# mathwrx/Decouple-and-Couple_Learning_in_Multi-Modal_Brain_Tumor_Segmentation

Measured on AMD Instinct MI355X. Metric: training volumes/sec (4x128^3), higher is better.
Workload: dtype bf16x3 forward (split-bf16 MFMA operands hi.hi+hi.lo+lo.hi: logits within 1e-3 of the fp32 reference) / bf16 data-gradient / bf16 weight-gradient MFMA operands; f32 accumulate, f32 storage, f32 master weights

## Files before the change

### decouple-and-couple_learning_in_multi-modal_brain_tumor_segmentation_amd/csrc/conv_args.h

```cpp
#pragma once
#include "common.h"

typedef __bf16 bf16x8 __attribute__((ext_vector_type(8)));
typedef unsigned u32x4 __attribute__((ext_vector_type(4)));

struct ConvArgsB {
  ConvGeom g;
  const float* x; const uint4* wpk; const float* bias; float* y;
  const float* in_scale; const float* in_shift; float in_slope;
  const float* residual; int r_ldc; const float* out_scale; double* stats;
  unsigned long long unused_[2];
  const float* nb_x; int nb_ldc; const float* nb_scale; const float* nb_shift; float nb_slope;
  int groups, x_goff, y_goff;
  const uint4* wpk_g[3]; const float* bias_g[3];
  const uint4* x16; const uint4* zero16;
  unsigned short* y16;
};

typedef __bf16 bf16x2_t __attribute__((ext_vector_type(2)));
typedef float f32x2_t __attribute__((ext_vector_type(2)));
__device__ __forceinline__ unsigned pack_bf16(float a, float b) {
  const f32x2_t f = {a, b};
  return __builtin_bit_cast(unsigned, __builtin_convertvector(f, bf16x2_t));
}
__device__ __forceinline__ float bf16_round(float a) { return (float)(__bf16)a; }
__device__ __forceinline__ void split_bf16(float a, float b, unsigned& hi, unsigned& lo) {
  hi = pack_bf16(a, b);
  const float ha = __builtin_bit_cast(float, hi << 16), hb = __builtin_bit_cast(float, hi & 0xffff0000u);
  lo = pack_bf16(a - ha, b - hb);
}
__device__ __forceinline__ float act01(float v, float slope) { return fmaxf(v, v * slope); }


static inline int cfg_extent(int op, int Di, int Hi, int Wi, int Do, int Ho, int Wo, int cd[3]) {
  cd[0] = Do; cd[1] = Ho; cd[2] = Wo;
  if (op == CWF_CONVT2) { cd[0] = Di; cd[1] = Hi; cd[2] = Wi; return 8; }
  if (op == CWF_CONV3_S2_DGRAD) { cd[0] = (Do + 1) / 2; cd[1] = (Ho + 1) / 2; cd[2] = (Wo + 1) / 2; return 8; }
  return 1;
}

int cwf_try_conv_ws(int op, int x3, ConvArgsB& a, hipStream_t st, int* rc);

int conv_fp32_launch(const cwf_conv_args& d, hipStream_t st);
int conv_stem_launch(const cwf_conv_args& d, hipStream_t st);
int conv_s2c16_launch(const cwf_conv_args& d, hipStream_t st);
int wgrad_fp32_launch(const cwf_wgrad_args& d, int* nsplit_used, hipStream_t st);
```

### decouple-and-couple_learning_in_multi-modal_brain_tumor_segmentation_amd/csrc/conv_bf16.hip

```cpp
#include "common.h"
#include <cstdio>
#include <cstdlib>
#include <type_traits>

#include "conv_args.h"

#define CB_MAXS 13
struct StageSlots { int goff[CB_MAXS]; unsigned inb; int nslots; };

__device__ __forceinline__ void stage_slots_init(StageSlots& ss, const ConvGeom& g, int id0, int ih0, int iw0, int tid) {
  const int nvox_in = g.ID * g.IH * g.IW;
  ss.nslots = (nvox_in + 63) >> 6; ss.inb = 0u;
  const int dq = 64 / g.IW, dr = 64 - dq * g.IW;
  int iw = (tid >> 2) % g.IW, t2 = (tid >> 2) / g.IW;
  int ih = t2 % g.IH, idd = t2 / g.IH;
#pragma unroll
  for (int i = 0; i < CB_MAXS; ++i) {
    const int v = (tid >> 2) + 64 * i;
    const int gd = id0 + idd, gh = ih0 + ih, gw = iw0 + iw;
    const bool ok = v < nvox_in && gd >= 0 && gd < g.Di && gh >= 0 && gh < g.Hi && gw >= 0 && gw < g.Wi;
    ss.goff[i] = ok ? ((gd * g.Hi + gh) * g.Wi + gw) * g.x_ldc : 0;
    ss.inb |= ok ? (1u << i) : 0u;
    iw += dr; int adv = dq;
    if (iw >= g.IW) { iw -= g.IW; ++adv; }
// ... 997 lines not shown
}

__global__ void gather_split_bf16_kernel(const cwf_gather_desc* __restrict__ table) {
  const cwf_gather_desc d = table[blockIdx.y];
  unsigned short* dst = reinterpret_cast<unsigned short*>(d.dst);
  const int64_t ngrp = d.n >> 3;
  const bool vec = ((d.n & 7) == 0) && ((reinterpret_cast<uintptr_t>(d.map) & 15) == 0) && ((reinterpret_cast<uintptr_t>(d.dst) & 15) == 0);
  if (vec) {
    for (int64_t gi = (int64_t)blockIdx.x * blockDim.x + threadIdx.x; gi < ngrp; gi += (int64_t)gridDim.x * blockDim.x) {
      const int4 m0 = *reinterpret_cast<const int4*>(d.map + gi * 8), m1 = *reinterpret_cast<const int4*>(d.map + gi * 8 + 4);
      const int mm[8] = {m0.x, m0.y, m0.z, m0.w, m1.x, m1.y, m1.z, m1.w};
      bool other = false;
#pragma unroll
      for (int e = 0; e < 8; ++e) other |= mm[e] == -2;
      unsigned short hh[8], ll[8];
#pragma unroll
      for (int e = 0; e < 8; ++e) {
        const float v = mm[e] >= 0 ? d.src[mm[e]] : 0.f;
        const __bf16 h = (__bf16)v;
        const __bf16 l = (__bf16)(v - (float)h);
        hh[e] = __builtin_bit_cast(unsigned short, h); ll[e] = __builtin_bit_cast(unsigned short, l);
      }
      unsigned short* o = dst + gi * 16;
      if (!other) {
        uint4 H, L;
        H.x = hh[0] | ((unsigned)hh[1] << 16); H.y = hh[2] | ((unsigned)hh[3] << 16); H.z = hh[4] | ((unsigned)hh[5] << 16); H.w = hh[6] | ((unsigned)hh[7] << 16);
        L.x = ll[0] | ((unsigned)ll[1] << 16); L.y = ll[2] | ((unsigned)ll[3] << 16); L.z = ll[4] | ((unsigned)ll[5] << 16); L.w = ll[6] | ((unsigned)ll[7] << 16);
        *reinterpret_cast<uint4*>(o) = H;
        *reinterpret_cast<uint4*>(o + 8) = L;
      } else {
#pragma unroll
        for (int e = 0; e < 8; ++e)
          if (mm[e] != -2) { o[e] = hh[e]; o[e + 8] = ll[e]; }
      }
    }
    return;
  }
  for (int64_t i = (int64_t)blockIdx.x * blockDim.x + threadIdx.x; i < d.n; i += (int64_t)gridDim.x * blockDim.x) {
    const int32_t m = d.map[i];
    if (m == -2) continue;
    const float v = m >= 0 ? d.src[m] : 0.f;
    const __bf16 h = (__bf16)v;
    const __bf16 l = (__bf16)(v - (float)h);
    const int64_t o = (i >> 3) * 16 + (i & 7);
    dst[o] = __builtin_bit_cast(unsigned short, h);
    dst[o + 8] = __builtin_bit_cast(unsigned short, l);
  }
}

extern "C" int cwf_gather_split_bf16(const struct cwf_gather_desc* table, int nlayers, int64_t max_n, void* stream) {
  if (!table || nlayers <= 0 || max_n <= 0) return CWF_E_BADARG;
  int64_t gx = cdiv64(max_n, 8 * 256); if (gx > 256) gx = 256; if (gx < 1) gx = 1;
  hipLaunchKernelGGL(gather_split_bf16_kernel, dim3((unsigned)gx, nlayers), dim3(256), 0, cwf_stream(stream), table);
  CWF_LAUNCH_CHECK();
  return 0;
}

namespace {
struct TileCfg { int MT, NT, WM; };
TileCfg choose_cfg(int op, const int cdims[3], int ncls, int N, int ntiles) {
  const bool s2 = (op == CWF_CONV3_S2 || op == CWF_CONVT2_DGRAD);
  static const TileCfg all[] = {{4, 4, 1}, {2, 4, 2}, {2, 4, 4}, {4, 2, 4}, {4, 1, 4}, {1, 4, 4}, {1, 2, 4}, {1, 2, 2}, {1, 1, 4}};
  TileCfg best = {1, 1, 4};
  double best_score = -1.0;
  for (const TileCfg& c : all) {
    const int WN = 4 / c.WM, MTOT = c.MT * c.WM, NTOT = c.NT * WN;
    if (s2 && MTOT > 4) continue;
    int TD, TH;
    switch (MTOT) { case 16: TD = 4; TH = 4; break; case 8: TD = 2; TH = 4; break; case 4: TD = 2; TH = 2; break; case 2: TD = 1; TH = 2; break; default: TD = 1; TH = 1; }
    const double sp_tiles = (double)cdiv(cdims[0], TD) * cdiv(cdims[1], TH) * cdiv(cdims[2], 16);
    const double sp_eff = ((double)cdims[0] * cdims[1] * cdims[2]) / (sp_tiles * MTOT * 16);
    const int ngrp = cdiv(ntiles, NTOT);
    const double n_eff = (double)ntiles / (ngrp * NTOT);
    const double nwg = sp_tiles * ngrp * N * ncls;
    const double fill = nwg >= 512 ? 1.0 : nwg / 512.0;
    const double reuse = 1.0 - 0.35 / (c.MT * c.NT) - 0.1 / MTOT;
    const double score = sp_eff * n_eff * fill * reuse;
    if (score > best_score) { best_score = score; best = c; }
  }
  return best;
}

template <int MT, int NT, int WM, bool X3>
int launch_cfg(const ConvArgsB& a, hipStream_t st) {
  constexpr int WN = 4 / WM;
  const ConvGeom& g = a.g;
  const size_t lds_tile = (size_t)g.ID * g.IH * g.IW * 16 * sizeof(unsigned short) * (X3 ? 2 : 1);
  const size_t lds_red = (size_t)4 * NT * 16 * 2 * sizeof(float);
  const size_t lds = lds_tile > lds_red ? lds_tile : lds_red;
  if (lds > 160 * 1024) return CWF_E_TOOLARGE;
  CWF_MAX_LDS_ONCE((&conv_bf16_kernel<MT, NT, WM, X3>));
  dim3 grid(g.tiles_d * g.tiles_h * g.tiles_w, cdiv(g.ntiles, WN * NT), g.N * g.ncls * (a.groups ? a.groups : 1));
  hipLaunchKernelGGL((conv_bf16_kernel<MT, NT, WM, X3>), grid, dim3(256), lds, st, a);
  CWF_LAUNCH_CHECK();
  return 0;
}
}

extern "C" int cwf_debug_conv_bf16_cfg(int op, int N, int Di, int Hi, int Wi, int Do, int Ho, int Wo, int Cout, int* mt_nt_wm) {
  if (!mt_nt_wm || N <= 0 || Di <= 0 || Hi <= 0 || Wi <= 0 || Do <= 0 || Ho <= 0 || Wo <= 0 || Cout <= 0 || op < CWF_CONV3_S1 ||
      op > CWF_CONVT2_DGRAD)
    return CWF_E_BADARG;
  int cd[3];
  const int ncls = cfg_extent(op, Di, Hi, Wi, Do, Ho, Wo, cd);
  const TileCfg c = choose_cfg(op, cd, ncls, N, cdiv(Cout, 16));
  mt_nt_wm[0] = c.MT; mt_nt_wm[1] = c.NT; mt_nt_wm[2] = c.WM;
  return 0;
}

static void c16_tap_order(ConvGeom& g) {
  int nat[27];
  for (int t = 0; t < 27; ++t) nat[t] = g.tapofs[t];
  for (int t = 0; t < 27; ++t) g.tapofs[t] = nat[c16_tap(t)];
}

static int conv_bf16_impl(const cwf_conv_args& d, hipStream_t st) {
  const int op = d.op, x3 = d.precision == CWF_BF16X3, N = d.N, Cin = d.Cin, Cout = d.Cout, y_ldc = d.y_ldc;
  const float* x = d.x16 ? reinterpret_cast<const float*>(d.x16) : d.x;
  const int x_ldc = d.x16 ? 16 : d.x_ldc;
  if (!x || !d.wpk || !d.y || N <= 0 || Cin <= 0 || Cout <= 0) return CWF_E_BADARG;
  if (d.nb_x && (!d.stats || !d.nb_scale || !d.nb_shift || d.nb_ldc < Cout)) return CWF_E_BADARG;
  if ((Cin & 3) || (x_ldc & 3) || x_ldc < Cin || y_ldc < Cout) return CWF_E_ALIGN;
  if (((uintptr_t)x & 15) || ((uintptr_t)d.wpk & 15)) return CWF_E_ALIGN;
  if (d.in_scale && !d.in_shift) return CWF_E_BADARG;
  ConvArgsB a;
  int cd[3];
  const int ncls = cfg_extent(op, d.Di, d.Hi, d.Wi, d.Do, d.Ho, d.Wo, cd);
  const TileCfg c = choose_cfg(op, cd, ncls, N, cdiv(Cout, 16));
  int rc = cwf_build_geom(a.g, op, N, d.Di, d.Hi, d.Wi, Cin, x_ldc, d.Do, d.Ho, d.Wo, Cout, y_ldc, c.MT * c.WM);
  if (rc) return rc;
  a.x = x; a.wpk = reinterpret_cast<const uint4*>(d.wpk); a.bias = d.bias; a.y = d.y; a.in_scale = d.in_scale; a.in_shift = d.in_shift;
  a.in_slope = d.x16 ? 1.f : d.in_slope; a.residual = d.residual; a.r_ldc = d.r_ldc; a.out_scale = d.out_scale; a.stats = d.stats;
  a.nb_x = d.nb_x; a.nb_ldc = d.nb_ldc; a.nb_scale = d.nb_scale; a.nb_shift = d.nb_shift; a.nb_slope = d.nb_x ? d.nb_slope : 1.f;
  a.groups = 0; a.x_goff = 0; a.y_goff = 0;
  a.x16 = reinterpret_cast<const uint4*>(d.x16); a.zero16 = reinterpret_cast<const uint4*>(d.zero16);
  a.y16 = reinterpret_cast<unsigned short*>(d.y16);
  for (int q = 0; q < 3; ++q) { a.wpk_g[q] = nullptr; a.bias_g[q] = nullptr; }
  if (d.x16) {
    c16_tap_order(a.g);
    rc = cwf_build_geom(a.g, op, N, d.Di, d.Hi, d.Wi, Cin, x_ldc, d.Do, d.Ho, d.Wo, Cout, y_ldc, 16);
    if (rc) return rc;
    return launch_conv16s<false, true>(a, st);
  }
  {
    int ks, nt;
    if (pw_eligible(op, a, &ks, &nt)) {
      if (d.y16 && (op != CWF_CONV1 || (Cout & 3) || ((uintptr_t)d.y16 & 7))) return CWF_E_BADARG;
      return x3 ? dispatch_pw<true>(op, a, st, ks, nt) : dispatch_pw<false>(op, a, st, ks, nt);
    }
    if (d.y16) return CWF_E_BADARG;
  }
  {
    int rcw = 0;
    if (cwf_try_conv_ws(op, x3, a, st, &rcw)) return rcw;
  }
  if (op == CWF_CONV3_S1 && Cin <= 16 && Cout <= 16) c16_tap_order(a.g);
  if (op == CWF_CONV3_S1 && Cin <= 16 && Cout <= 16 && (int64_t)d.Do * d.Ho * d.Wo >= 32768) {
    rc = cwf_build_geom(a.g, op, N, d.Di, d.Hi, d.Wi, Cin, x_ldc, d.Do, d.Ho, d.Wo, Cout, y_ldc, 16);
    if (rc) return rc;
    return x3 ? launch_conv16s<true>(a, st) : launch_conv16s<false>(a, st);
  }
#define CWF_CFG(mt, nt, wm) if (c.MT == mt && c.NT == nt && c.WM == wm) return x3 ? launch_cfg<mt, nt, wm, true>(a, st) : launch_cfg<mt, nt, wm, false>(a, st);
  CWF_CFG(4, 4, 1) CWF_CFG(2, 4, 2) CWF_CFG(2, 4, 4) CWF_CFG(4, 2, 4) CWF_CFG(4, 1, 4)
  CWF_CFG(1, 4, 4) CWF_CFG(1, 2, 4) CWF_CFG(1, 2, 2) CWF_CFG(1, 1, 4)
#undef CWF_CFG
  return CWF_E_BADARG;
}

static int conv_grouped_impl(const cwf_conv_args& d, hipStream_t st) {
  const int op = d.op, x3 = d.precision == CWF_BF16X3, groups = d.groups, N = d.N, Cin = d.Cin, Cout = d.Cout;
  const int x_ldc = d.x_ldc, y_ldc = d.y_ldc, x_goff = d.x_goff, y_goff = d.y_goff;
  if (!d.x || !d.y || N <= 0 || Cin <= 0 || Cout <= 0) return CWF_E_BADARG;
  if ((Cin & 3) || (x_ldc & 3) || (x_goff & 3) || x_ldc < (groups - 1) * x_goff + Cin || y_ldc < (groups - 1) * y_goff + Cout) return CWF_E_ALIGN;
  if ((uintptr_t)d.x & 15) return CWF_E_ALIGN;
  ConvArgsB a;
  int cd[3];
  TileCfg c = choose_cfg(op, cd, cfg_extent(op, d.Di, d.Hi, d.Wi, d.Do, d.Ho, d.Wo, cd), N * groups, cdiv(Cout, 16));
  int rc = cwf_build_geom(a.g, op, N, d.Di, d.Hi, d.Wi, Cin, x_ldc, d.Do, d.Ho, d.Wo, Cout, y_ldc, c.MT * c.WM);
  if (rc) return rc;
  a.x = d.x; a.wpk = nullptr; a.bias = nullptr; a.y = d.y; a.in_scale = nullptr; a.in_shift = nullptr; a.in_slope = 1.f;
  a.residual = nullptr; a.r_ldc = 0; a.out_scale = nullptr; a.stats = nullptr;
  a.nb_x = nullptr; a.nb_ldc = 0; a.nb_scale = nullptr; a.nb_shift = nullptr; a.nb_slope = 1.f;
  a.groups = groups; a.x_goff = x_goff; a.y_goff = y_goff;
  a.x16 = nullptr; a.zero16 = nullptr; a.y16 = nullptr;
  for (int q = 0; q < 3; ++q) {
    a.wpk_g[q] = q < groups ? reinterpret_cast<const uint4*>(d.wpk_g[q]) : nullptr;
    a.bias_g[q] = q < groups ? d.bias_g[q] : nullptr;
    if (q < groups && (!d.wpk_g[q] || ((uintptr_t)d.wpk_g[q] & 15))) return CWF_E_ALIGN;
  }
  if (Cin <= 16 && Cout <= 16) c16_tap_order(a.g);
#define CWF_CFG(mt, nt, wm) if (c.MT == mt && c.NT == nt && c.WM == wm) return x3 ? launch_cfg<mt, nt, wm, true>(a, st) : launch_cfg<mt, nt, wm, false>(a, st);
  CWF_CFG(4, 4, 1) CWF_CFG(2, 4, 2) CWF_CFG(2, 4, 4) CWF_CFG(4, 2, 4) CWF_CFG(4, 1, 4)
  CWF_CFG(1, 4, 4) CWF_CFG(1, 2, 4) CWF_CFG(1, 2, 2) CWF_CFG(1, 1, 4)
#undef CWF_CFG
  return CWF_E_BADARG;
}

extern "C" int cwf_conv(const struct cwf_conv_args* args, void* stream) {
  if (!args) return CWF_E_BADARG;
  const cwf_conv_args& d = *args;
  if (d.precision != CWF_FP32 && d.precision != CWF_BF16X3 && d.precision != CWF_BF16) return CWF_E_BADARG;
  const bool fp32 = d.precision == CWF_FP32;
  hipStream_t st = cwf_stream(stream);
  if (d.groups) {
    if (d.groups < 2 || d.groups > 3 || d.op != CWF_CONV3_S1 || d.in_scale || d.residual || d.out_scale || d.stats || d.nb_x || d.x16 ||
        d.y16 || d.w_raw)
      return CWF_E_BADARG;
    if (!fp32) return conv_grouped_impl(d, st);
    for (int q = 0; q < d.groups; ++q) {
      cwf_conv_args g = d;
      g.groups = 0; g.x = d.x + q * d.x_goff; g.y = d.y + q * d.y_goff; g.wpk = d.wpk_g[q]; g.bias = d.bias_g[q];
      const int rc = conv_fp32_launch(g, st);
      if (rc) return rc;
    }
    return 0;
  }
  if (d.x16) {
    if (d.precision != CWF_BF16 || d.in_scale || d.out_scale || d.y16 || !d.zero16 || ((uintptr_t)d.x16 & 15) || ((uintptr_t)d.zero16 & 15))
      return CWF_E_BADARG;
    if (d.op != CWF_CONV3_S1 || d.Cin != 16 || d.Cout != 16 || d.Do != d.Di || d.Ho != d.Hi || d.Wo != d.Wi ||
        (int64_t)d.Di * d.Hi * d.Wi < 32768 || (int64_t)d.N * d.Di * d.Hi * d.Wi >= (1ll << 30))
      return CWF_E_BADARG;
    return conv_bf16_impl(d, st);
  }
  if (d.y16) {
    if (d.nb_x || d.out_scale) return CWF_E_BADARG;
    if (!fp32 && d.op == CWF_CONV1) {
      const int rc = conv_bf16_impl(d, st);
      if (rc != CWF_E_BADARG) return rc;
    }
    cwf_conv_args f = d;
    f.y16 = nullptr;
    const int rc = cwf_conv(&f, stream);
    if (rc) return rc;
    return cwf_to_bf16(d.y, d.y_ldc, nullptr, nullptr, 1.f, d.y16, d.N, (int64_t)d.Do * d.Ho * d.Wo, d.Cout, stream);
  }
  const int64_t vo = (int64_t)d.Do * d.Ho * d.Wo;
  if (d.w_raw && !fp32 && !d.in_scale && !d.residual && !d.nb_x) {
    if (d.op == CWF_CONV3_S1 && d.Cin == 4 && d.Cout == 16 && vo >= 32768) return conv_stem_launch(d, st);
    if (d.op == CWF_CONV3_S2 && d.Cin == 16 && d.Cout == 32 && !d.out_scale && vo >= 32768 &&
        d.Do == (d.Di + 1) / 2 && d.Ho == (d.Hi + 1) / 2 && d.Wo == (d.Wi + 1) / 2)
      return conv_s2c16_launch(d, st);
  }
  if (fp32) return d.nb_x ? CWF_E_BADARG : conv_fp32_launch(d, st);
  return conv_bf16_impl(d, st);
}
```

### decouple-and-couple_learning_in_multi-modal_brain_tumor_segmentation_amd/csrc/conv_ws.hip

```cpp
#include "conv_args.h"
#include <cstdlib>
#include <type_traits>

#define WS_ID 6
#define WS_IH 6
#define WS_IW 18
#define WS_NVOX (WS_ID * WS_IH * WS_IW)
#define WS_SLOTS 11
#define WS_NT 2

struct WsWork { int ngroups, slots, tiles, xcd_perm; };

__host__ __device__ constexpr int ws_tap_bytes(int t) { return (((t / 9) * WS_IH + (t / 3) % 3) * WS_IW + t % 3) * 32; }

template <bool X3>
__global__ __launch_bounds__(512) void convws_kernel(const ConvArgsB a, const WsWork wk) {
  constexpr int NT = WS_NT;
  constexpr int T = 1;
  extern __shared__ float4 lds4[];
  const ConvGeom& g = a.g;
  const int nch = g.nchunks;
  char* lds = reinterpret_cast<char*>(lds4);
  constexpr int B_IMG = 14 * NT * 1024;
  constexpr int B_ALL = B_IMG * (X3 ? 2 : 1);
// ... 224 lines not shown
    const char* bl = Bl + b_lane;
    const char* ah0 = Ah + a_lane;
    const char* al0 = Al + a_lane;
    uint4 fa[2][4], fb[2][NT], fl[4], fbl[NT];
    auto rd_hi = [&](auto S, auto P) {
      constexpr int s = decltype(S)::value, p = decltype(P)::value;
      constexpr int c0 = ws_tap_bytes(2 * s), c1 = ws_tap_bytes(2 * s + 1 < 27 ? 2 * s + 1 : 2 * s);
      const int to = second ? c1 : c0;
#pragma unroll
      for (int m = 0; m < 4; ++m) fa[p][m] = *reinterpret_cast<const uint4*>(ah0 + to + m * (WS_IW * 32));
#pragma unroll
      for (int j = 0; j < NT; ++j) fb[p][j] = *reinterpret_cast<const uint4*>(bh + (s * NT + j) * 1024);
    };
    auto rd_lo = [&](auto S) {
      constexpr int s = decltype(S)::value;
      constexpr int c0 = ws_tap_bytes(2 * s), c1 = ws_tap_bytes(2 * s + 1 < 27 ? 2 * s + 1 : 2 * s);
      const int to = second ? c1 : c0;
#pragma unroll
      for (int m = 0; m < 4; ++m) fl[m] = *reinterpret_cast<const uint4*>(al0 + to + m * (WS_IW * 32));
#pragma unroll
      for (int j = 0; j < NT; ++j) fbl[j] = *reinterpret_cast<const uint4*>(bl + (s * NT + j) * 1024);
    };
    auto mm = [&](auto P) {
      constexpr int p = decltype(P)::value;
#pragma unroll
      for (int m = 0; m < 4; ++m)
#pragma unroll
        for (int j = 0; j < NT; ++j)
          acc[k][m][j] = __builtin_amdgcn_mfma_f32_16x16x32_bf16(__builtin_bit_cast(bf16x8, fa[p][m]), __builtin_bit_cast(bf16x8, fb[p][j]), acc[k][m][j], 0, 0, 0);
      if (X3) {
#pragma unroll
        for (int m = 0; m < 4; ++m)
#pragma unroll
          for (int j = 0; j < NT; ++j)
            acc[k][m][j] = __builtin_amdgcn_mfma_f32_16x16x32_bf16(__builtin_bit_cast(bf16x8, fa[p][m]), __builtin_bit_cast(bf16x8, fbl[j]), acc[k][m][j], 0, 0, 0);
#pragma unroll
        for (int m = 0; m < 4; ++m)
#pragma unroll
          for (int j = 0; j < NT; ++j)
            acc[k][m][j] = __builtin_amdgcn_mfma_f32_16x16x32_bf16(__builtin_bit_cast(bf16x8, fl[m]), __builtin_bit_cast(bf16x8, fb[p][j]), acc[k][m][j], 0, 0, 0);
      }
    };
    using I0 = std::integral_constant<int, 0>; using I1 = std::integral_constant<int, 1>;
#define WS_IC(v) std::integral_constant<int, (v)>{}
#define WS_STEP2(S0)                                                                                           \
    if (X3) rd_lo(WS_IC(S0)); rd_hi(WS_IC((S0) + 1), I1{}); mm(I0{}); __builtin_amdgcn_sched_barrier(0);       \
    if (X3) rd_lo(WS_IC((S0) + 1)); if ((S0) + 2 < 14) rd_hi(WS_IC((S0) + 2 < 14 ? (S0) + 2 : 13), I0{});      \
    mm(I1{}); __builtin_amdgcn_sched_barrier(0);
    rd_hi(I0{}, I0{});
    WS_STEP2(0) WS_STEP2(2) WS_STEP2(4) WS_STEP2(6) WS_STEP2(8) WS_STEP2(10) WS_STEP2(12)
#undef WS_STEP2
#undef WS_IC
    if (chunk == nch - 1) { epilogue(tile, KK); return true; }
    return false;
  };
  using K0 = std::integral_constant<int, 0>;
  auto do_issue = [&](int blk) {
    const int round = blk / nch, tile = item_tile(round, 0);
    if (tile >= 0) issue_loads(tile, blk - round * nch);
  };
  auto do_convert = [&](int blk, int younger) {
    const int round = blk / nch, tile = item_tile(round, 0);
    if (tile < 0) return;
    (void)younger;
    asm volatile("" : "+v"(pf_sc), "+v"(pf_sh));
    convert_write(tile, blk - round * nch, pf_sc, pf_sh);
  };
  if (n_blocks > 0) {
    do_issue(0);
    if (grp == 0) {
      b_issue(0);
      do_convert(0, -1);
      __syncthreads();
      b_write();
      __syncthreads();
      for (int blk = 0; blk < n_blocks; ++blk) {
        const bool more = blk + 1 < n_blocks;
        if (more) do_issue(blk + 1);
        const bool epi = mfma_item(blk, K0{});
        __syncthreads();
        if (more) {
          b_issue((blk + 1) % nch);
          do_convert(blk + 1, NB + (epi ? 32 : 0));
        }
        __syncthreads();
        if (more) {
          b_write();
          __syncthreads();
        }
      }
    } else {
      __syncthreads();
      __syncthreads();
      do_convert(0, -1);
      for (int blk = 0; blk < n_blocks; ++blk) {
        const bool more = blk + 1 < n_blocks;
        __syncthreads();
        if (more) do_issue(blk + 1);
        const bool epi = mfma_item(blk, K0{});
        __syncthreads();
        if (more) {
          __syncthreads();
          do_convert(blk + 1, epi ? 32 : 0);
        }
      }
    }
  }

  if (a.stats) {
#pragma unroll
    for (int j = 0; j < NT; ++j) {
      float u1 = s1[j], u2 = s2[j];
      u1 += __shfl_xor(u1, 16, 64); u1 += __shfl_xor(u1, 32, 64);
      u2 += __shfl_xor(u2, 16, 64); u2 += __shfl_xor(u2, 32, 64);
      if (kq == 0) {
        red[((wave * NT + j) * 16 + r) * 2 + 0] = u1;
        red[((wave * NT + j) * 16 + r) * 2 + 1] = u2;
      }
    }
    int* red_n = reinterpret_cast<int*>(red + 8 * NT * 16 * 2);
    if (lane == 0) red_n[wave] = stats_n;
    __syncthreads();
    if (tid < 2 * NT * 16 * 2) {
      const int gsel = tid / (NT * 16 * 2), t2 = tid % (NT * 16 * 2);
      const int which = t2 & 1, rr = (t2 >> 1) & 15, jj = t2 >> 5;
      const int sn = red_n[gsel * 4];
      if (sn >= 0) {
        double s = 0.0;
#pragma unroll
        for (int w = 0; w < 4; ++w) s += (double)red[(((gsel * 4 + w) * NT + jj) * 16 + rr) * 2 + which];
        const int co = (nt0 + jj) * 16 + rr;
        atomic_add_f64(a.stats + ((int64_t)sn * g.Cout + co) * 2 + which, s);
      }
    }
  }
}

namespace {
template <bool X3>
int launch_ws(const ConvArgsB& a, const WsWork& wk, int grid, hipStream_t st) {
  const size_t lds = (size_t)14 * WS_NT * 1024 * (X3 ? 2 : 1) + (size_t)2 * WS_NVOX * 32 * (X3 ? 2 : 1) + 8 * WS_NT * 16 * 2 * sizeof(float) + 64;
  if (lds > 160 * 1024) return CWF_E_TOOLARGE;
  CWF_MAX_LDS_ONCE((&convws_kernel<X3>));
  hipLaunchKernelGGL((convws_kernel<X3>), dim3(grid), dim3(512), lds, st, a, wk);
  CWF_LAUNCH_CHECK();
  return 0;
}
}

static int g_ws_min_units = 256;
extern "C" int cwf_debug_ws_min_units(int v) { const int old = g_ws_min_units; g_ws_min_units = v; return old; }
static int g_ws_x3 = 0;
extern "C" int cwf_debug_ws_x3(int v) { const int old = g_ws_x3; g_ws_x3 = v; return old; }

int cwf_try_conv_ws(int op, int x3, ConvArgsB& a, hipStream_t st, int* rc) {
  const ConvGeom& g = a.g;
  if (op != CWF_CONV3_S1 || a.groups || a.out_scale || (x3 && !g_ws_x3)) return 0;
  if (g.Cin < 32 || (g.Cin & 15) || (g.Cout & 31)) return 0;
  if ((g.Do & 3) || (g.Ho & 3) || (g.Wo & 15)) return 0;
  if (g.x_ldc < g.Cin || (g.x_ldc & 3)) return 0;
  WsWork wk;
  wk.ngroups = g.Cout / 32;
  if (wk.ngroups > 32) return 0;
  const int64_t tiles = (int64_t)g.N * (g.Do / 4) * (g.Ho / 4) * (g.Wo / 16);
  if (tiles * wk.ngroups < g_ws_min_units) return 0;
  int e = cwf_build_geom(a.g, op, g.N, g.Di, g.Hi, g.Wi, g.Cin, g.x_ldc, g.Do, g.Ho, g.Wo, g.Cout, g.y_ldc, 16);
  if (e) { *rc = e; return 1; }
  wk.tiles = (int)tiles;
  int per = (32 / wk.ngroups) * wk.ngroups;
  wk.slots = 8 * (per / wk.ngroups);
  wk.xcd_perm = 1;
  if (wk.slots * 2 > wk.tiles) { wk.slots = (wk.tiles + 1) / 2; wk.xcd_perm = 0; }
  const int grid = wk.slots * wk.ngroups;
  *rc = x3 ? launch_ws<true>(a, wk, grid, st) : launch_ws<false>(a, wk, grid, st);
  return 1;
}
```

Measured before the change: 113.9.

## Add warp-specialized persistent split-bf16 3x3x3 conv kernel for the bf16x3 forward

Adds a new persistent, warp-specialized kernel for stride-1 3x3x3 convolutions in the bf16x3 (split hi/lo) forward path. Four producer waves load activations, apply the input norm and activation, split them into hi/lo bf16 and stage them in double-buffered LDS along with hi/lo weights. Four consumer waves run the three MFMA passes and a fused bias/residual/stats epilogue. Each block processes a slice of tiles and can hold up to four tiles' accumulators, so it avoids the staged-tile kernels' per-tile setup and overlaps loads with MFMA. The cost is higher register and LDS pressure, and statistics are now reduced in a different order. It is gated to Cin at or above 128 and to enough work units.

Result: faster. 115.9 (median of 6 runs) (+1.8%).

```diff
diff --git a/decouple-and-couple_learning_in_multi-modal_brain_tumor_segmentation_amd/csrc/conv_args.h b/decouple-and-couple_learning_in_multi-modal_brain_tumor_segmentation_amd/csrc/conv_args.h
--- a/decouple-and-couple_learning_in_multi-modal_brain_tumor_segmentation_amd/csrc/conv_args.h
+++ b/decouple-and-couple_learning_in_multi-modal_brain_tumor_segmentation_amd/csrc/conv_args.h
@@ -40,6 +40,8 @@
 }
 
 int cwf_try_conv_ws(int op, int x3, ConvArgsB& a, hipStream_t st, int* rc);
+int cwf_ws_takes_x3();
+int cwf_try_conv_wsp(int op, int x3, int cfg_mt, int cfg_wm, ConvArgsB& a, hipStream_t st, int* rc);
 
 int conv_fp32_launch(const cwf_conv_args& d, hipStream_t st);
 int conv_stem_launch(const cwf_conv_args& d, hipStream_t st);
diff --git a/decouple-and-couple_learning_in_multi-modal_brain_tumor_segmentation_amd/csrc/conv_bf16.hip b/decouple-and-couple_learning_in_multi-modal_brain_tumor_segmentation_amd/csrc/conv_bf16.hip
--- a/decouple-and-couple_learning_in_multi-modal_brain_tumor_segmentation_amd/csrc/conv_bf16.hip
+++ b/decouple-and-couple_learning_in_multi-modal_brain_tumor_segmentation_amd/csrc/conv_bf16.hip
@@ -1173,6 +1173,7 @@
   }
   {
     int rcw = 0;
+    if (cwf_try_conv_wsp(op, x3, c.MT, c.WM, a, st, &rcw)) return rcw;
     if (cwf_try_conv_ws(op, x3, a, st, &rcw)) return rcw;
   }
   if (op == CWF_CONV3_S1 && Cin <= 16 && Cout <= 16) c16_tap_order(a.g);
diff --git a/decouple-and-couple_learning_in_multi-modal_brain_tumor_segmentation_amd/csrc/conv_ws.hip b/decouple-and-couple_learning_in_multi-modal_brain_tumor_segmentation_amd/csrc/conv_ws.hip
--- a/decouple-and-couple_learning_in_multi-modal_brain_tumor_segmentation_amd/csrc/conv_ws.hip
+++ b/decouple-and-couple_learning_in_multi-modal_brain_tumor_segmentation_amd/csrc/conv_ws.hip
@@ -400,6 +400,7 @@
 extern "C" int cwf_debug_ws_min_units(int v) { const int old = g_ws_min_units; g_ws_min_units = v; return old; }
 static int g_ws_x3 = 0;
 extern "C" int cwf_debug_ws_x3(int v) { const int old = g_ws_x3; g_ws_x3 = v; return old; }
+int cwf_ws_takes_x3() { return g_ws_x3; }
 
 int cwf_try_conv_ws(int op, int x3, ConvArgsB& a, hipStream_t st, int* rc) {
   const ConvGeom& g = a.g;
diff --git a/decouple-and-couple_learning_in_multi-modal_brain_tumor_segmentation_amd/csrc/conv_wsp.hip b/decouple-and-couple_learning_in_multi-modal_brain_tumor_segmentation_amd/csrc/conv_wsp.hip
--- /dev/null
+++ b/decouple-and-couple_learning_in_multi-modal_brain_tumor_segmentation_amd/csrc/conv_wsp.hip
@@ -0,0 +1,387 @@
+#include "conv_args.h"
+#include <cstdlib>
+#include <type_traits>
+
+#define WSP_ID 6
+#define WSP_IH 6
+#define WSP_IW 18
+#define WSP_NVOX (WSP_ID * WSP_IH * WSP_IW)
+#define WSP_SLOTS 11
+#define WSP_NT 2
+#define WSP_NBW 14
+
+struct WspWork { int ngroups, slots, tiles, xcd_perm, stat_rows; };
+
+__host__ __device__ constexpr int wsp_tap_bytes(int t) { return (((t / 9) * WSP_IH + (t / 3) % 3) * WSP_IW + t % 3) * 32; }
+
+template <int T>
+__global__ __launch_bounds__(512) void convwsp_kernel(const ConvArgsB a, const WspWork wk) {
+  constexpr int NT = WSP_NT;
+  constexpr int B_IMG = 14 * NT * 1024;
+  constexpr int A_IMG = WSP_NVOX * 32;
+  constexpr int A_BUF = 2 * A_IMG;
+  extern __shared__ float4 lds4[];
+  char* lds = reinterpret_cast<char*>(lds4);
+  char* const Bh = lds;
+  char* const Bl = lds + B_IMG;
+  char* const A0 = lds + 2 * B_IMG;
+  const ConvGeom& g = a.g;
+  const int nch = g.nchunks;
+  const int tid = threadIdx.x, lane = tid & 63;
+  const int wave = __builtin_amdgcn_readfirstlane(tid >> 6);
+
+  int cgrp, slot;
+  {
+    const int b = blockIdx.x;
+    if (wk.xcd_perm) {
+      const int per = gridDim.x >> 3, j = b >> 3;
+      cgrp = j % wk.ngroups;
+      slot = (b & 7) * (per / wk.ngroups) + j / wk.ngroups;
+    } else {
+      cgrp = b % wk.ngroups;
+      slot = b / wk.ngroups;
+    }
+  }
+  const int t_begin = (int)(((int64_t)slot * wk.tiles) / wk.slots), t_end = (int)(((int64_t)(slot + 1) * wk.tiles) / wk.slots);
+  const int ntw = t_end - t_begin;
+  const int nt0 = cgrp * NT;
+  const int tiles_per_n = g.tiles_d * g.tiles_h * g.tiles_w;
+
+  if (wave < 4) {
+    const int wl = wave;
+    const int r = lane & 15, kq = lane >> 4;
+    const bool second = (kq >> 1) != 0;
+    const int a_lane = ((wl * WSP_IH) * WSP_IW + r) * 32 + (kq & 1) * 16;
+    const int b_lane = lane * 16;
+
+    f32x4 acc[T][4][NT];
+#pragma unroll
+    for (int k = 0; k < T; ++k)
+#pragma unroll
+      for (int m = 0; m < 4; ++m)
+#pragma unroll
+        for (int j = 0; j < NT; ++j) acc[k][m][j] = (f32x4){0.f, 0.f, 0.f, 0.f};
+    float s1[NT], s2[NT];
+    double d1[NT], d2[NT];
+#pragma unroll
+    for (int j = 0; j < NT; ++j) { s1[j] = 0.f; s2[j] = 0.f; d1[j] = 0.0; d2[j] = 0.0; }
+    int stats_n = -1;
+    auto fold_stats = [&]() {
+#pragma unroll
+      for (int j = 0; j < NT; ++j) {
+        float u1 = s1[j], u2 = s2[j];
+        u1 += __shfl_xor(u1, 16, 64); u1 += __shfl_xor(u1, 32, 64);
+        u2 += __shfl_xor(u2, 16, 64); u2 += __shfl_xor(u2, 32, 64);
+        d1[j] += (double)u1; d2[j] += (double)u2;
+        s1[j] = 0.f; s2[j] = 0.f;
+      }
+    };
+    auto flush_stats = [&]() {
+#pragma unroll
+      for (int j = 0; j < NT; ++j) {
+        if (kq == 0) {
+          const int co = (nt0 + j) * 16 + r;
+          atomic_add_f64(a.stats + ((int64_t)stats_n * g.Cout + co) * 2 + 0, d1[j]);
+          atomic_add_f64(a.stats + ((int64_t)stats_n * g.Cout + co) * 2 + 1, d2[j]);
+        }
+        d1[j] = 0.0; d2[j] = 0.0;
+      }
+    };
+
+    auto epilogue = [&](int tile, auto KK) {
+      constexpr int k = decltype(KK)::value;
+      const int n = tile / tiles_per_n;
+      int bx = tile - n * tiles_per_n;
+      const int tw = bx % g.tiles_w; bx /= g.tiles_w;
+      const int th = bx % g.tiles_h, td = bx / g.tiles_h;
+      if (a.stats && n != stats_n) {
+        if (stats_n >= 0) flush_stats();
+        stats_n = n;
+      }
+      float bvj[NT];
+#pragma unroll
+      for (int j = 0; j < NT; ++j) bvj[j] = a.bias ? a.bias[(nt0 + j) * 16 + r] : 0.f;
+      auto epi = [&](auto HR, auto HT) {
+        constexpr bool HAS_RES = decltype(HR)::value, HAS_STATS = decltype(HT)::value;
+        unsigned yo[4], ro[4];
+#pragma unroll
+        for (int i = 0; i < 4; ++i) {
+          yo[i] = (unsigned)((kq * 4 + i) * g.y_ldc + nt0 * 16 + r) * 4u; asm volatile("" : "+v"(yo[i]));
+          if (HAS_RES) { ro[i] = (unsigned)((kq * 4 + i) * a.r_ldc + nt0 * 16 + r) * 4u; asm volatile("" : "+v"(ro[i])); }
+        }
+        const int od = td * 4 + wl;
+        float rv[4][NT][4];
+        if (HAS_RES) {
+#pragma unroll
+          for (int m = 0; m < 4; ++m) {
+            const int64_t vox0 = (((int64_t)n * g.Do + od) * g.Ho + th * 4 + m) * g.Wo + tw * 16;
+            const char* rb = reinterpret_cast<const char*>(a.residual + vox0 * a.r_ldc);
+#pragma unroll
+            for (int j = 0; j < NT; ++j)
+#pragma unroll
+              for (int i = 0; i < 4; ++i) rv[m][j][i] = *reinterpret_cast<const float*>(rb + ro[i] + j * 64);
+          }
+        }
+#pragma unroll
+        for (int m = 0; m < 4; ++m) {
+          const int64_t vox0 = (((int64_t)n * g.Do + od) * g.Ho + th * 4 + m) * g.Wo + tw * 16;
+          char* yb = reinterpret_cast<char*>(a.y + vox0 * g.y_ldc);
+#pragma unroll
+          for (int j = 0; j < NT; ++j)
+#pragma unroll
+            for (int i = 0; i < 4; ++i) {
+              float v = acc[k][m][j][i] + bvj[j];
+              if (HAS_RES) v += rv[m][j][i];
+              *reinterpret_cast<float*>(yb + yo[i] + j * 64) = v;
+              if (HAS_STATS) { s1[j] += v; s2[j] = fmaf(v, v, s2[j]); }
+              acc[k][m][j][i] = 0.f;
+            }
+          if (HAS_STATS && (wk.stat_rows == 1 || m == 3)) fold_stats();
+        }
+      };
+      using T_ = std::true_type; using F_ = std::false_type;
+      if (a.residual) { if (a.stats) epi(T_{}, T_{}); else epi(T_{}, F_{}); }
+      else            { if (a.stats) epi(F_{}, T_{}); else epi(F_{}, F_{}); }
+    };
+
+    auto mfma_item = [&](int buf, auto KK) {
+      constexpr int k = decltype(KK)::value;
+      const char* bh = Bh + b_lane;
+      const char* bl = Bl + b_lane;
+      const char* ah0 = A0 + buf * A_BUF + a_lane;
+      const char* al0 = ah0 + A_IMG;
+      uint4 fa[2][4], fb[2][NT], fl[4], fbl[NT];
+      auto rd_hi = [&](auto S, auto P) {
+        constexpr int s = decltype(S)::value, p = decltype(P)::value;
+        constexpr int c0 = wsp_tap_bytes(2 * s), c1 = wsp_tap_bytes(2 * s + 1 < 27 ? 2 * s + 1 : 2 * s);
+        const int to = second ? c1 : c0;
+#pragma unroll
+        for (int m = 0; m < 4; ++m) fa[p][m] = *reinterpret_cast<const uint4*>(ah0 + to + m * (WSP_IW * 32));
+#pragma unroll
+        for (int j = 0; j < NT; ++j) fb[p][j] = *reinterpret_cast<const uint4*>(bh + (s * NT + j) * 1024);
+      };
+      auto rd_lo = [&](auto S) {
+        constexpr int s = decltype(S)::value;
+        constexpr int c0 = wsp_tap_bytes(2 * s), c1 = wsp_tap_bytes(2 * s + 1 < 27 ? 2 * s + 1 : 2 * s);
+        const int to = second ? c1 : c0;
+#pragma unroll
+        for (int m = 0; m < 4; ++m) fl[m] = *reinterpret_cast<const uint4*>(al0 + to + m * (WSP_IW * 32));
+#pragma unroll
+        for (int j = 0; j < NT; ++j) fbl[j] = *reinterpret_cast<const uint4*>(bl + (s * NT + j) * 1024);
+      };
+      auto mm = [&](auto P) {
+        constexpr int p = decltype(P)::value;
+#pragma unroll
+        for (int m = 0; m < 4; ++m)
+#pragma unroll
+          for (int j = 0; j < NT; ++j)
+            acc[k][m][j] = __builtin_amdgcn_mfma_f32_16x16x32_bf16(__builtin_bit_cast(bf16x8, fa[p][m]), __builtin_bit_cast(bf16x8, fb[p][j]), acc[k][m][j], 0, 0, 0);
+#pragma unroll
+        for (int m = 0; m < 4; ++m)
+#pragma unroll
+          for (int j = 0; j < NT; ++j)
+            acc[k][m][j] = __builtin_amdgcn_mfma_f32_16x16x32_bf16(__builtin_bit_cast(bf16x8, fa[p][m]), __builtin_bit_cast(bf16x8, fbl[j]), acc[k][m][j], 0, 0, 0);
+#pragma unroll
+        for (int m = 0; m < 4; ++m)
+#pragma unroll
+          for (int j = 0; j < NT; ++j)
+            acc[k][m][j] = __builtin_amdgcn_mfma_f32_16x16x32_bf16(__builtin_bit_cast(bf16x8, fl[m]), __builtin_bit_cast(bf16x8, fb[p][j]), acc[k][m][j], 0, 0, 0);
+      };
+      using I0 = std::integral_constant<int, 0>; using I1 = std::integral_constant<int, 1>;
+#define WSP_IC(v) std::integral_constant<int, (v)>{}
+#define WSP_STEP2(S0)                                                                                          \
+      rd_lo(WSP_IC(S0)); rd_hi(WSP_IC((S0) + 1), I1{}); mm(I0{}); __builtin_amdgcn_sched_barrier(0);            \
+      rd_lo(WSP_IC((S0) + 1)); if ((S0) + 2 < 14) rd_hi(WSP_IC((S0) + 2 < 14 ? (S0) + 2 : 13), I0{});           \
+      mm(I1{}); __builtin_amdgcn_sched_barrier(0);
+      rd_hi(I0{}, I0{});
+      WSP_STEP2(0) WSP_STEP2(2) WSP_STEP2(4) WSP_STEP2(6) WSP_STEP2(8) WSP_STEP2(10) WSP_STEP2(12)
+#undef WSP_STEP2
+#undef WSP_IC
+    };
+
+    int i = 0;
+    for (int t0 = 0; t0 < ntw; t0 += T) {
+      const int nk = min(T, ntw - t0);
+      for (int c = 0; c < nch; ++c) {
+        auto item = [&](auto KK) {
+          constexpr int k = decltype(KK)::value;
+          if (k == 0 && i > 0) asm volatile("s_barrier" ::: "memory");
+          asm volatile("s_barrier" ::: "memory");
+          mfma_item(i & 1, KK);
+          if (c == nch - 1) epilogue(t_begin + t0 + k, KK);
+          ++i;
+        };
+        item(std::integral_constant<int, 0>{});
+        if (T > 1 && nk > 1) item(std::integral_constant<int, (T > 1 ? 1 : 0)>{});
+        if (T > 2 && nk > 2) item(std::integral_constant<int, (T > 2 ? 2 : 0)>{});
+        if (T > 3 && nk > 3) item(std::integral_constant<int, (T > 3 ? 3 : 0)>{});
+      }
+    }
+    if (a.stats && stats_n >= 0) flush_stats();
+  } else {
+    const int tg = tid - 256;
+    const int ni = ntw * nch;
+    struct Item { int tile, chunk; bool first; };
+    auto item_of = [&](int it) {
+      const int per_round = T * nch;
+      const int rd = it / per_round, w = it - rd * per_round;
+      const int nk = min(T, ntw - rd * T);
+      const int c = w / nk, k = w - c * nk;
+      Item o; o.tile = t_begin + rd * T + k; o.chunk = c; o.first = k == 0;
+      return o;
+    };
+
+    u32x4 wpf[WSP_NBW];
+    const uint4* wsrc = a.wpk + (int64_t)g.cls_wbase16[0] * 128;
+    auto w_issue = [&](int chunk) {
+      int tgo = tg;
+      asm volatile("" : "+v"(tgo));
+#pragma unroll
+      for (int i = 0; i < WSP_NBW; ++i) {
+        const int e = tgo + 256 * i;
+        const int img = e / (14 * NT * 64), e2 = e - img * (14 * NT * 64);
+        const int ln = e2 & 63, blk = e2 >> 6;
+        const int j = blk % NT, s = blk / NT;
+        const uint4* p = wsrc + ((int64_t)(chunk * 14 + s) * g.ntiles + nt0 + j) * 128 + ln * 2 + img;
+        wpf[i] = *reinterpret_cast<const u32x4*>(p);
+      }
+    };
+    auto w_write = [&]() {
+      int wb = tg * 16;
+      asm volatile("" : "+v"(wb));
+#pragma unroll
+      for (int i = 0; i < WSP_NBW; ++i) *reinterpret_cast<u32x4*>(Bh + wb + i * 4096) = wpf[i];
+    };
+
+    const int q = tg & 3;
+    const int vox0 = tg >> 2;
+    const int iw_0 = vox0 % WSP_IW, row_0 = vox0 / WSP_IW;
+    const bool plain = a.in_scale == nullptr && a.in_slope == 1.f;
+    f32x4 pf[WSP_SLOTS];
+    f32x4 pf_sc, pf_sh;
+    unsigned pf_inb = 0u;
+    auto issue = [&](int it) {
+      const Item itm = item_of(it);
+      const int tile = itm.tile, chunk = itm.chunk;
+      const int n = tile / tiles_per_n;
+      int bx = tile - n * tiles_per_n;
+      const int tw = bx % g.tiles_w; bx /= g.tiles_w;
+      const int th = bx % g.tiles_h, td = bx / g.tiles_h;
+      const int id0 = td * 4 - 1, ih0 = th * 4 - 1, iw0 = tw * 16 - 1;
+      const char* xb = reinterpret_cast<const char*>(a.x + (int64_t)n * g.Di * g.Hi * g.Wi * g.x_ldc + chunk * 16);
+      const unsigned ldc4 = (unsigned)g.x_ldc * 4u;
+      unsigned inb = 0u;
+      int iw = iw_0, row = row_0;
+      asm volatile("" : "+v"(iw), "+v"(row));
+#pragma unroll
+      for (int i = 0; i < WSP_SLOTS; ++i) {
+        const int idd = (row * 43) >> 8, ih = row - idd * WSP_IH;
+        const int gd = id0 + idd, gh = ih0 + ih, gw = iw0 + iw;
+        const bool ok = (row < WSP_ID * WSP_IH) & ((unsigned)gd < (unsigned)g.Di) & ((unsigned)gh < (unsigned)g.Hi) & ((unsigned)gw < (unsigned)g.Wi);
+        iw += 10; row += 3;
+        if (iw >= WSP_IW) { iw -= WSP_IW; ++row; }
+        const unsigned lin = (unsigned)((gd * g.Hi + gh) * g.Wi + gw) * ldc4 + (unsigned)q * 16u;
+        const unsigned boff = ok ? lin : (unsigned)q * 16u;
+        pf[i] = *reinterpret_cast<const f32x4*>(xb + boff);
+        inb |= ok ? (1u << i) : 0u;
+      }
+      pf_inb = inb;
+      const float* scp = a.in_scale ? a.in_scale + (int64_t)n * g.Cin + chunk * 16 : a.x;
+      const float* shp = a.in_scale ? a.in_shift + (int64_t)n * g.Cin + chunk * 16 : a.x;
+      pf_sc = *reinterpret_cast<const f32x4*>(reinterpret_cast<const char*>(scp) + q * 16);
+      pf_sh = *reinterpret_cast<const f32x4*>(reinterpret_cast<const char*>(shp) + q * 16);
+    };
+    auto convert = [&](int buf) {
+      const float slope = a.in_slope;
+      const bool has_norm = a.in_scale != nullptr;
+      const f32x4 sc = has_norm ? pf_sc : (f32x4){1.f, 1.f, 1.f, 1.f}, sh = has_norm ? pf_sh : (f32x4){0.f, 0.f, 0.f, 0.f};
+      const unsigned inb = pf_inb;
+      int vbase = (tg >> 2) * 32 + q * 8;
+      asm volatile("" : "+v"(vbase));
+      char* ah = A0 + buf * A_BUF + vbase;
+#pragma unroll
+      for (int i = 0; i < WSP_SLOTS; ++i) {
+        if (i == WSP_SLOTS - 1 && vox0 + 64 * i >= WSP_NVOX) continue;
+        float v0 = pf[i][0], v1 = pf[i][1], v2 = pf[i][2], v3 = pf[i][3];
+        if (!plain) {
+          v0 = act01(fmaf(v0, sc[0], sh[0]), slope); v1 = act01(fmaf(v1, sc[1], sh[1]), slope);
+          v2 = act01(fmaf(v2, sc[2], sh[2]), slope); v3 = act01(fmaf(v3, sc[3], sh[3]), slope);
+        }
+        uint2 h, l;
+        split_bf16(v0, v1, h.x, l.x); split_bf16(v2, v3, h.y, l.y);
+        const bool was = (inb >> i) & 1u;
+        h.x = was ? h.x : 0u; h.y = was ? h.y : 0u; l.x = was ? l.x : 0u; l.y = was ? l.y : 0u;
+        *reinterpret_cast<uint2*>(ah + i * (64 * 32)) = h;
+        *reinterpret_cast<uint2*>(ah + A_IMG + i * (64 * 32)) = l;
+      }
+    };
+
+    __builtin_amdgcn_s_setprio(1);
+    if (ni > 0) {
+      issue(0);
+      w_issue(0);
+      convert(0);
+      w_write();
+      if (ni > 1) issue(1);
+    }
+    for (int it = 0; it < ni; ++it) {
+      if (it > 0 && item_of(it).first) {
+        asm volatile("s_barrier" ::: "memory");
+        w_write();
+      }
+      asm volatile("s_waitcnt lgkmcnt(0)\n\ts_barrier" ::: "memory");
+      if (it + 1 < ni) {
+        convert((it + 1) & 1);
+        const Item nx = item_of(it + 1);
+        if (nx.first) w_issue(nx.chunk);
+        if (it + 2 < ni) issue(it + 2);
+      }
+    }
+  }
+}
+
+namespace {
+template <int T>
+int launch_wsp(const ConvArgsB& a, const WspWork& wk, int grid, hipStream_t st) {
+  const size_t lds = (size_t)2 * 14 * WSP_NT * 1024 + (size_t)2 * 2 * WSP_NVOX * 32;
+  CWF_MAX_LDS_ONCE((&convwsp_kernel<T>));
+  hipLaunchKernelGGL((convwsp_kernel<T>), dim3(grid), dim3(512), lds, st, a, wk);
+  CWF_LAUNCH_CHECK();
+  return 0;
+}
+}
+
+static int g_wsp = 1;
+extern "C" int cwf_debug_wsp(int v) { const int old = g_wsp; g_wsp = v; return old; }
+static long long g_wsp_launches = 0;
+extern "C" long long cwf_debug_wsp_launches() { return g_wsp_launches; }
+static const int g_wsp_min_cin = 128, g_wsp_min_units = 128;
+
+int cwf_try_conv_wsp(int op, int x3, int cfg_mt, int cfg_wm, ConvArgsB& a, hipStream_t st, int* rc) {
+  const ConvGeom& g = a.g;
+  if (!g_wsp || !x3 || cwf_ws_takes_x3()) return 0;
+  if (op != CWF_CONV3_S1 || a.groups || a.out_scale || a.nb_x) return 0;
+  if (g.Cin < 32 || (g.Cin & 15) || (g.Cout & 31)) return 0;
+  if ((g.Do & 3) || (g.Ho & 3) || (g.Wo & 15)) return 0;
+  if (g.x_ldc < g.Cin || (g.x_ldc & 3)) return 0;
+  if ((int64_t)g.Di * g.Hi * g.Wi * g.x_ldc * 4 >= (1ll << 31)) return 0;
+  if (a.stats && !(cfg_mt == 1 || (cfg_mt == 4 && cfg_wm == 4))) return 0;
+  WspWork wk;
+  wk.stat_rows = cfg_mt;
+  wk.ngroups = g.Cout / 32;
+  if (wk.ngroups > 32) return 0;
+  const int64_t tiles = (int64_t)g.N * (g.Do / 4) * (g.Ho / 4) * (g.Wo / 16);
+  if (g_wsp == 1 && (g.Cin < g_wsp_min_cin || tiles * wk.ngroups < g_wsp_min_units)) return 0;
+  int e = cwf_build_geom(a.g, op, g.N, g.Di, g.Hi, g.Wi, g.Cin, g.x_ldc, g.Do, g.Ho, g.Wo, g.Cout, g.y_ldc, 16);
+  if (e) { *rc = e; return 1; }
+  wk.tiles = (int)tiles;
+  const int per = (32 / wk.ngroups) * wk.ngroups;
+  wk.slots = 8 * (per / wk.ngroups);
+  wk.xcd_perm = 1;
+  if (wk.slots > wk.tiles) { wk.slots = wk.tiles; wk.xcd_perm = 0; }
+  const int grid = wk.slots * wk.ngroups;
+  const int per_wg = (wk.tiles + wk.slots - 1) / wk.slots;
+  *rc = per_wg > 2 ? launch_wsp<4>(a, wk, grid, st) : launch_wsp<2>(a, wk, grid, st);
+  if (*rc == 0) ++g_wsp_launches;
+  return 1;
+}
```
